# jw007123/hp-Adaptive-Signed-Distance-Field-Octree

Hardware: AMD Instinct MI355X
Metric: Query() Mpts/sec at targetError=1e-5 (union3 field, 10M SplitMix64 pts per GPU, HBM-resident); Create() ms reported as create_ms (higher is better)
Workload: dtype f64

## Files before the change

### hp-adaptive-signed-distance-field-octree_amd/csrc/fit.hip

```cpp
#include <hip/hip_runtime.h>

#include <algorithm>
#include <cstdint>
#include <cstdlib>

#include "device_types.hpp"
#include "fit_kernels.hpp"
#include "launch.hpp"
#include "leaf_eval.hpp"

namespace hpsdf {

__global__ __launch_bounds__(256) void pack_kernel(const PackItem* __restrict__ items, uint32_t nItems,
                                                   const double* __restrict__ arena, double* __restrict__ out) {
    const uint32_t wave = (blockIdx.x * blockDim.x + threadIdx.x) >> 6, lane = threadIdx.x & 63;
    if (wave >= nItems) return;
    const PackItem it = items[wave];
    for (uint32_t i = lane; i < it.count; i += 64) out[it.dst + i] = arena[it.src + i];
}

size_t fitLdsBytes(int degree, int nTasks, int planes) {
    const size_t nq = 4 * (size_t)degree + 1;
    return ((size_t)(degree + 1) * nq + 2 * nq + 8 * (size_t)nTasks + (size_t)nTasks * planes * nq * nq) * sizeof(double);
}
// ... 32 lines not shown
        sh.planes = std::max(sh.planes, std::min(nq, minPlanes));
        while (sh.cells > 1 && fitLdsBytes(degree, sh.cells, sh.planes) > kFitMaxLdsBytes) --sh.cells;
        sh.ldsBytes = fitLdsBytes(degree, sh.cells, sh.planes);
    }
    return sh;
}

#define HPSDF_DISPATCH_KIND(FN, field, ...)                          \
    switch ((field).kind) {                                          \
        case kFieldAnalytic: FN<kFieldAnalytic>(__VA_ARGS__); break; \
        case kFieldSamples: FN<kFieldSamples>(__VA_ARGS__); break;   \
        default: FN<kFieldMesh>(__VA_ARGS__); break;                 \
    }

hipError_t launchFitMulti(hipStream_t stream, const FitBlock* dBlocks, uint32_t maxBlocks, size_t ldsBytes, const FitTask* dTasks,
                          double* dArena, double* dErrs, const DeviceTables* dTables, const FieldDev& field, const RootMap& rm,
                          const uint32_t* dCount) {
    if (maxBlocks == 0) return hipSuccess;
    if (ldsBytes > kFitMaxLdsBytes) return hipErrorInvalidValue;
    HPSDF_DISPATCH_KIND(launchFitMultiKind, field, stream, dBlocks, maxBlocks, ldsBytes, dTasks, dArena, dErrs, dTables, field, rm, dCount);
    return hipGetLastError();
}

hipError_t launchFit(hipStream_t stream, int degree, int cellsPerThread, const FitBlock* dBlocks, uint32_t nBlocks,
                     size_t ldsBytes, const FitTask* dTasks, double* dArena, double* dErrs, double* dMirror,
                     const DeviceTables* dTables, const FieldDev& field, const RootMap& rm, const uint32_t* dRange) {
    if (nBlocks == 0) return hipSuccess;
    if (ldsBytes > kFitMaxLdsBytes) return hipErrorInvalidValue;
    HPSDF_DISPATCH_KIND(launchFitKind, field, stream, degree, cellsPerThread, dBlocks, nBlocks, ldsBytes, dTasks, dArena,
                        dErrs, dMirror, dTables, field, rm, dRange);
    return hipGetLastError();
}

hipError_t launchFieldEval(hipStream_t stream, const FieldDev& f, const DeviceTables* dTables, const double* dXyz,
                           size_t n, double* dOut) {
    if (n == 0) return hipSuccess;
    HPSDF_DISPATCH_KIND(launchFieldKind, f, stream, f, dTables, dXyz, n, dOut);
    return hipGetLastError();
}

hipError_t launchPack(hipStream_t stream, const PackItem* dItems, uint32_t nItems, const double* dArena, double* dOut) {
    if (nItems == 0) return hipSuccess;
    const unsigned blocks = (nItems + 3) / 4;
    hipLaunchKernelGGL(pack_kernel, dim3(blocks), dim3(256), 0, stream, dItems, nItems, dArena, dOut);
    return hipGetLastError();
}

}
```

### hp-adaptive-signed-distance-field-octree_amd/csrc/fit_analytic.hip

```cpp
#include "fit_kernels.hpp"

namespace hpsdf {

HPSDF_FIT_KIND_UNIT(, kFieldAnalytic)

}
```

### hp-adaptive-signed-distance-field-octree_amd/csrc/fit_kernels.hpp

```cpp
#pragma once
#include <hip/hip_runtime.h>

#include <cstdint>

#include "device_types.hpp"
#include "field_glue.hpp"
#include "launch.hpp"

namespace hpsdf {


constexpr int kFitPiece = 8;
#ifndef HPSDF_FIT_MIN_WAVES
#define HPSDF_FIT_MIN_WAVES 4
#endif

__device__ __forceinline__ double fitRowAny(double acc, double a1, const double* __restrict__ tk, double n2,
                                            const double* __restrict__ F, int nq) {
    int k = 0;
    for (; k + 4 <= nq; k += 4) {
        const double f0 = F[k], f1 = F[k + 1], f2 = F[k + 2], f3 = F[k + 3];
        const double t0 = tk[k], t1 = tk[k + 1], t2 = tk[k + 2], t3 = tk[k + 3];
        acc = acc + (a1 * t0 * n2) * f0;
        acc = acc + (a1 * t1 * n2) * f1;
        acc = acc + (a1 * t2 * n2) * f2;
        acc = acc + (a1 * t3 * n2) * f3;
    }
    for (; k < nq; ++k) acc = acc + (a1 * tk[k] * n2) * F[k];
    return acc;
}

template <int KIND, bool CSG, int DEG, int R, bool LEFT>
__device__ __forceinline__ void fitBlockBody(const FitBlock blk, const FitTask* __restrict__ tasks, double* __restrict__ arena,
                                             double* __restrict__ errs, double* __restrict__ mirror,
                                             const DeviceTables* __restrict__ T, const FieldDev& field, const RootMap& rm, double* lds) {
    static_assert(R == 1 || DEG > 0, "cell blocking needs a compile-time degree");
    __shared__ double sNl[13 * 11];
    __shared__ double sRec[26];
    __shared__ int32_t sMeshStack[kFitThreads / 64][kMeshStack];
    __shared__ unsigned char sPosI[KIND == kFieldMesh ? 64 : 4], sPosJK[KIND == kFieldMesh ? 64 : 4];
    const int tid = threadIdx.x;
    const int deg = DEG > 0 ? DEG : (int)blk.degree;
    const int nq = 4 * deg + 1, nq2 = nq * nq, G = blk.nTasks;
    const int rowStart = blk.rowStart, rowEnd = blk.rowEnd, nrows = rowEnd - rowStart;
    const int gl = nq * (nq - 1) / 2;
    const int planes = blk.planesPerChunk;
    const int depth = blk.depth;
    const bool split = blk.split != 0;

    double* sT = lds;
    double* sR = sT + (deg + 1) * nq;
    double* sW = sR + nq;
    double* sC = sW + nq;
    double* sF = sC + 8 * G;

    stageQueryTables(T, sNl, sRec);
    for (int q = tid; q < nq; q += kFitThreads) {
        const double x = T->roots[gl + q];
        sR[q] = x;
        sW[q] = T->weights[gl + q];
        double m2 = 0.0, m1 = 1.0;
        sT[q] = 1.0;
        for (int i = 1; i <= deg; ++i) {
            const double l = T->rec[i][0] * x * m1 - T->rec[i][1] * m2;
            m2 = m1, m1 = l;
// ... 189 lines not shown
    const int outBase = split ? 0 : stashBase;
    if (act0) {
#pragma unroll
        for (int r = 0; r < R; ++r)
            if (g2 + r < G) {
                const uint64_t at = tasks[blk.firstTask + g2 + r].outOff + (r0 - outBase);
                arena[at] = acc[r];
                if (mirror != nullptr) mirror[at] = acc[r];
                sF[(g2 + r) * stashStride + (r0 - stashBase)] = acc[r];
            }
    }
    if (act1) {
        arena[tasks[blk.firstTask].outOff + (r1 - outBase)] = acc1;
        sF[r1 - stashBase] = acc1;
    }
    if (weighted && rowStart > 0) {
        for (int s = tid; s < G * rowStart; s += kFitThreads) {
            const int g = s / rowStart, r = s - g * rowStart;
            const FitTask& tk = tasks[blk.firstTask + g];
            const double v = arena[tk.copyOff + r];
            arena[tk.outOff + r] = v;
            sF[g * stashStride + r] = v;
        }
    }
    __syncthreads();
    for (int g = tid; g < G; g += kFitThreads) {
        const int first = deg > 0 ? (int)T->count[deg - 1] : 0;
        double e = 0.0;
        for (int r = first > rowStart ? first : rowStart; r < rowEnd; ++r)
            if (T->bidx[r][3] == deg) {
                const double c = sF[g * stashStride + (r - stashBase)];
                e = e + c * c;
            }
        errs[tasks[blk.firstTask + g].errSlot] = e;
    }
}

template <int KIND, bool CSG, bool LEFT>
__global__ __launch_bounds__(kFitThreads, HPSDF_FIT_MIN_WAVES) void fit_multi_kernel(const FitBlock* __restrict__ blocks,
                                                                const FitTask* __restrict__ tasks, double* __restrict__ arena,
                                                                double* __restrict__ errs, const DeviceTables* __restrict__ T,
                                                                FieldDev field, RootMap rm, const uint32_t* __restrict__ count,
                                                                uint32_t countValue) {
    extern __shared__ double lds[];
    const uint32_t n = count ? *count : countValue;
    if (blockIdx.x >= n) return;
    const FitBlock blk = blocks[n - 1u - blockIdx.x];
    switch (blk.degree) {
        case 2: fitBlockBody<KIND, CSG, 2, 1, LEFT>(blk, tasks, arena, errs, nullptr, T, field, rm, lds); break;
        case 3: fitBlockBody<KIND, CSG, 3, 1, LEFT>(blk, tasks, arena, errs, nullptr, T, field, rm, lds); break;
        case 4: fitBlockBody<KIND, CSG, 4, 1, LEFT>(blk, tasks, arena, errs, nullptr, T, field, rm, lds); break;
        case 5: fitBlockBody<KIND, CSG, 5, 1, LEFT>(blk, tasks, arena, errs, nullptr, T, field, rm, lds); break;
        case 6: fitBlockBody<KIND, CSG, 6, 1, LEFT>(blk, tasks, arena, errs, nullptr, T, field, rm, lds); break;
        case 7: fitBlockBody<KIND, CSG, 7, 1, LEFT>(blk, tasks, arena, errs, nullptr, T, field, rm, lds); break;
        case 8: fitBlockBody<KIND, CSG, 8, 1, LEFT>(blk, tasks, arena, errs, nullptr, T, field, rm, lds); break;
        default: fitBlockBody<KIND, CSG, 0, 1, LEFT>(blk, tasks, arena, errs, nullptr, T, field, rm, lds); break;
    }
}

template <int KIND, bool CSG, int DEG, int R, bool LEFT>
__global__ __launch_bounds__(kFitThreads, HPSDF_FIT_MIN_WAVES) void fit_kernel(const FitBlock* __restrict__ blocks,
                                                          const FitTask* __restrict__ tasks, double* __restrict__ arena,
                                                          double* __restrict__ errs, double* __restrict__ mirror,
                                                          const DeviceTables* __restrict__ T, FieldDev field, RootMap rm,
                                                          const uint32_t* __restrict__ range) {
    extern __shared__ double lds[];
    uint32_t b = blockIdx.x;
    if (range != nullptr) {
// ... 22 lines not shown
                       const DeviceTables* dTables, const FieldDev& field, const RootMap& rm, const uint32_t* dRange) {
#define HPSDF_FIT_LAUNCH(D, RR)                                                                                       \
    hipLaunchKernelGGL((fit_kernel<KIND, CSG, D, RR, LEFT>), dim3(nBlocks), dim3(kFitThreads), ldsBytes, stream, dBlocks, \
                       dTasks, dArena, dErrs, dMeans, dTables, field, rm, dRange)
#define HPSDF_FIT_CASE(D)       \
    case D:                     \
        HPSDF_FIT_LAUNCH(D, 1); \
        break;
    if (cellsPerThread != 1 && cellsPerThread != 4) cellsPerThread = 1;
    switch (degree) {
        HPSDF_FIT_CASE(2)
        HPSDF_FIT_CASE(3)
        HPSDF_FIT_CASE(4)
        HPSDF_FIT_CASE(5)
        HPSDF_FIT_CASE(6)
        HPSDF_FIT_CASE(7)
        HPSDF_FIT_CASE(8)
        default:
            HPSDF_FIT_LAUNCH(0, 1);
    }
#undef HPSDF_FIT_CASE
#undef HPSDF_FIT_LAUNCH
}

template <int KIND, bool CSG, bool LEFT>
static void launchFitMultiT(hipStream_t stream, const FitBlock* dBlocks, uint32_t maxBlocks, size_t ldsBytes, const FitTask* dTasks,
                            double* dArena, double* dErrs, const DeviceTables* dTables, const FieldDev& field, const RootMap& rm,
                            const uint32_t* dCount) {
    hipLaunchKernelGGL((fit_multi_kernel<KIND, CSG, LEFT>), dim3(maxBlocks), dim3(kFitThreads), ldsBytes, stream, dBlocks, dTasks, dArena, dErrs,
                       dTables, field, rm, dCount, maxBlocks);
}

template <int KIND, bool CSG, bool LEFT>
static void launchFieldT(hipStream_t stream, const FieldDev& f, const DeviceTables* dTables, const double* dXyz,
                         size_t n, double* dOut) {
    hipLaunchKernelGGL((field_kernel<KIND, CSG, LEFT>), dim3(gridFor(n)), dim3(256), 0, stream, f, dTables, dXyz, n, dOut);
}

#define HPSDF_DISPATCH_FIELD_ORDER(FN, K, C, field, ...)  \
    do {                                                  \
        if ((field).leftAssoc) FN<K, C, true>(__VA_ARGS__); \
        else FN<K, C, false>(__VA_ARGS__);                \
    } while (0)
#define HPSDF_DISPATCH_FIELD(FN, K, field, ...)                                                  \
    do {                                                                                         \
        if ((field).csgOp >= 0) HPSDF_DISPATCH_FIELD_ORDER(FN, K, true, field, __VA_ARGS__);     \
        else HPSDF_DISPATCH_FIELD_ORDER(FN, K, false, field, __VA_ARGS__);                       \
    } while (0)

template <int KIND>
void launchFitKind(hipStream_t stream, int degree, int cellsPerThread, const FitBlock* dBlocks, uint32_t nBlocks, size_t ldsBytes,
                   const FitTask* dTasks, double* dArena, double* dErrs, double* dMirror, const DeviceTables* dTables,
                   const FieldDev& field, const RootMap& rm, const uint32_t* dRange) {
    HPSDF_DISPATCH_FIELD(launchFitT, KIND, field, stream, degree, cellsPerThread, dBlocks, nBlocks, ldsBytes, dTasks, dArena,
                         dErrs, dMirror, dTables, field, rm, dRange);
}
template <int KIND>
void launchFitMultiKind(hipStream_t stream, const FitBlock* dBlocks, uint32_t maxBlocks, size_t ldsBytes, const FitTask* dTasks,
                        double* dArena, double* dErrs, const DeviceTables* dTables, const FieldDev& field, const RootMap& rm,
                        const uint32_t* dCount) {
    HPSDF_DISPATCH_FIELD(launchFitMultiT, KIND, field, stream, dBlocks, maxBlocks, ldsBytes, dTasks, dArena, dErrs, dTables, field, rm, dCount);
}
template <int KIND>
void launchFieldKind(hipStream_t stream, const FieldDev& f, const DeviceTables* dTables, const double* dXyz, size_t n, double* dOut) {
    HPSDF_DISPATCH_FIELD(launchFieldT, KIND, f, stream, f, dTables, dXyz, n, dOut);
}
#undef HPSDF_DISPATCH_FIELD
#undef HPSDF_DISPATCH_FIELD_ORDER

#define HPSDF_FIT_KIND_UNIT(EXTERN, K)                                                                                                 \
    EXTERN template void launchFitKind<K>(hipStream_t, int, int, const FitBlock*, uint32_t, size_t, const FitTask*, double*, double*, \
                                          double*, const DeviceTables*, const FieldDev&, const RootMap&, const uint32_t*);            \
    EXTERN template void launchFitMultiKind<K>(hipStream_t, const FitBlock*, uint32_t, size_t, const FitTask*, double*, double*,      \
                                               const DeviceTables*, const FieldDev&, const RootMap&, const uint32_t*);                \
    EXTERN template void launchFieldKind<K>(hipStream_t, const FieldDev&, const DeviceTables*, const double*, size_t, double*);
HPSDF_FIT_KIND_UNIT(extern, kFieldAnalytic)
HPSDF_FIT_KIND_UNIT(extern, kFieldSamples)
HPSDF_FIT_KIND_UNIT(extern, kFieldMesh)

}
```

### hp-adaptive-signed-distance-field-octree_amd/csrc/fit_samples.hip

```cpp
#include "fit_kernels.hpp"

namespace hpsdf {

HPSDF_FIT_KIND_UNIT(, kFieldSamples)

}
```

### hp-adaptive-signed-distance-field-octree_amd/csrc/frontier.hip

```cpp
#include <hip/hip_runtime.h>

#include <algorithm>
#include <atomic>
#include <cfloat>
#include <cmath>
#include <cstddef>
#include <chrono>
#include <cstdio>
#include <cstdlib>
#include <cstring>
#include <memory>
#include <vector>

#include "builder.hpp"
#include "frontier.hpp"
#include "launch.hpp"
#include "runtime.hpp"

namespace hpsdf {

namespace {

constexpr uint32_t kFrJobs = 4096;
constexpr uint32_t kFrTasks = 9 * kFrJobs;
// ... 5 lines not shown
constexpr uint32_t kFrSort = 4096;
constexpr uint32_t kFrExact = 64;
constexpr uint32_t kFrStatusPad = 8;

struct FrHdr {
    uint32_t nNodes, nQueued, nJobs, done;
    uint32_t round, maxDegree, maxDepth, overflow;
    uint32_t nTasks, nBlocks, takenCount, candCount;
    uint32_t above;
    int32_t t1;
    uint32_t nLeaves, arrive;
    uint32_t degBlocks[13][2];
    uint32_t degTasks[13][2];
    uint32_t lowTasks[13][2];
    uint64_t arenaUsed, sampleUsed, nCoeffs, pad1;
    uint64_t jobs, pRefines, hRefines, dropped, fits, samples;
    uint64_t splitFits;
    uint32_t splitRound, padR;
    uint64_t roundBase, partStride;
    double total, target;
    uint32_t rP, rH, rD, rMaxDeg;
    uint32_t rOps, rPad;
    uint32_t sliceFirst[9];
    uint32_t padS;
    uint64_t packCount[8];
    uint64_t dbg[24];
    int64_t rCoeffDelta;
    double rTotal;
    uint32_t opsArrive, stuck;
    uint32_t chainStamp;
    uint32_t landed;
    uint32_t stored[2];
    uint32_t storeArrive[2];
    uint32_t hist1[2048];
    uint32_t hist2[2048];
    uint64_t agg[kFrJobs / 128];
};
constexpr size_t kFrHdrCopyBytes = offsetof(FrHdr, hist1);
static_assert(kFrHdrCopyBytes / 4 <= 1024, "frMirror copies the header with one thread a word");
static inline void frCpuRelax() {
#if defined(__x86_64__) || defined(__i386__)
    __builtin_ia32_pause();
#elif defined(__aarch64__)
    asm volatile("yield");
#endif
}

struct FrRound {
    uint32_t cCount[kFrClasses], cFirst[kFrClasses], cCursor[kFrClasses], cBlockFirst[kFrClasses], cBlocks[kFrClasses];
    uint64_t cArena[kFrClasses], cSample[kFrClasses];
    uint64_t cArenaO[8][kFrClasses];
    uint8_t cG[kFrClasses], cPlanes[kFrClasses];
    uint64_t arenaBase;
};

struct FrDev {
    FrHdr* hdr;
    FrHdr* hostHdr;
    FrRound* rnd;
    hpsdf_node* nodes;
    uint64_t* qErr;
    uint32_t* parent;
    uint64_t* segOff;
    uint8_t* segFirst;
    uint32_t* sub;
    uint32_t* taken;
// ... 1127 lines not shown
                        if (b + 2u < batches) {
                            FR_CHAIN_LOAD(ra, b + 2u)
                        }
                        __builtin_amdgcn_sched_barrier(0);
                        FR_CHAIN_ADD(rb)
                    }
                    if (b < batches) {
                        FR_CHAIN_ADD(ra)
                    }
#undef FR_CHAIN_LOAD
#undef FR_CHAIN_ADD
                    t = batches << 4;
                }
                for (; t < steps; ++t) total = __builtin_amdgcn_mfma_f64_4x4x4f64(mine[4u * t], 1.0, total, 0, 0, 0);
                q = steps << 2;
            }
            for (; q < n; ++q) total = total + src[q];
            if (d.stamps && tid == 0 && c0 == 0) d.hdr->dbg[16] = __builtin_readcyclecounter();
        }
        __syncthreads();
    }
    if (tid == 0) sOps[0] = total;
    __syncthreads();
    return sOps[0];
}

__device__ void frChainTotal(const FrDev& d, FrLds& L, bool chain0) {
    FrHdr* h = d.hdr;
    const uint32_t tid = threadIdx.x, wave = tid >> 6;
    if (wave != 0 && (wave & 3u) == 0) return;
    const uint32_t stamp = h->round + 1u;
    const bool round0 = stamp == 1u;
    double total = h->total;
    if (tid == 0) L.stuck = 0;
    __syncthreads();
    const uint32_t nJobs0 = h->nJobs;
    if (tid == 0) __hip_atomic_fetch_add(&h->arrive, 1u, __ATOMIC_RELAXED, __HIP_MEMORY_SCOPE_AGENT);
    if (round0 && !chain0) return;
    uint32_t nOps = nJobs0;
    if (!round0) {
        if (tid == 0 && !frWaitAtLeast(&h->opsArrive, gridDim.x - 2u)) L.stuck = 1;
        __syncthreads();
        nOps = frLoad(&h->rP) + 9u * frLoad(&h->rH);
        if (L.stuck) nOps = 0;
    }
    if (d.stamps && tid == 0) h->dbg[13] = __builtin_readcyclecounter();
    total = frRunChain(d, L, total, nOps, round0);
    if (tid == 0) {
        if (d.stamps) h->dbg[14] = __builtin_readcyclecounter();
        if (L.stuck) atomicExch(&h->stuck, 1u);
        h->rTotal = total;
        frRelease();
        __hip_atomic_store(&h->chainStamp, stamp, __ATOMIC_RELAXED, __HIP_MEMORY_SCOPE_AGENT);
    }
}

__device__ void frLeadRound(const FrDev& d, FrLds& L, int pre, bool chain0) {
    FrHdr* h = d.hdr;
    const uint32_t tid = threadIdx.x, nJobs = h->nJobs, round = h->round, stamp = round + 1u;
    const bool round0 = round == 0;
    const uint32_t nNodes0 = h->nNodes, nQ0 = h->nQueued;
    const uint64_t jobs0 = h->jobs, pRef0 = h->pRefines, hRef0 = h->hRefines, drop0 = h->dropped, nCoeffs0 = h->nCoeffs;
    const uint32_t nLeaves0 = h->nLeaves, maxDeg0 = h->maxDegree;
    const uint64_t fits0 = h->fits, samples0 = h->samples, arena0 = h->arenaUsed, split0 = h->splitFits;
    const double target = d.target;
    if (tid == 0) L.flag = 0, L.stuck = 0;
    if (tid == 0 && round0) {
        *(volatile uint32_t*)&d.hostHdr->landed = d.buildStamp;
        __threadfence_system();
    }
    __syncthreads();
    frPeerCheck(d, &L.flag);
    FR_STAMP(9);
    double total0 = 0.0;
    const bool ownChain = round0 && !chain0;
    if (ownChain) {
        if (d.stamps && tid == 0) h->dbg[13] = __builtin_readcyclecounter();
        total0 = frRunChain(d, L, h->total, nJobs, true);
        if (d.stamps && tid == 0) h->dbg[14] = __builtin_readcyclecounter();
    }
    if (tid == 0 && !frWaitAtLeast(&h->arrive, gridDim.x - 1u)) L.stuck = 1;
    __syncthreads();
    FR_STAMP(10);
    const uint32_t nP = frLoad(&h->rP), nH = frLoad(&h->rH), nD = frLoad(&h->rD), md = frLoad(&h->rMaxDeg);
    const long long cd = (long long)__hip_atomic_load(reinterpret_cast<unsigned long long*>(&h->rCoeffDelta), __ATOMIC_RELAXED, __HIP_MEMORY_SCOPE_AGENT);
    uint32_t overflow = frLoad(&h->overflow) | ((L.stuck || frLoad(&h->stuck)) ? 4u : 0u);
    const uint32_t nQ = nQ0 - (round0 ? 0u : nJobs) + nP + 8u * nH;
    const uint32_t nNodes = nNodes0 + 8u * nH;
    const bool stopsHere = ownChain && total0 < target;
    if (!stopsHere)
        for (uint32_t i = tid; i < 2048; i += 1024) L.hist[i] = frLoad(&h->hist1[i]);
    if (tid == 0) {
        const bool there = !ownChain && frLoad(&h->chainStamp) == stamp;
        if (there) frAcquire();
        L.c = (ownChain || there) ? 1u : 0u;
    }
    __syncthreads();
    bool haveTotal = L.c != 0;
    const bool canGoOn = nQ != 0 && overflow == 0;
    if (canGoOn && nQ > d.K && !stopsHere) {
        frThreshold(L.hist, d.K, L.tmp, &L.t, &L.above);
    } else {
        if (tid == 0) L.t = -1, L.above = nQ;
        __syncthreads();
    }
    const int T = L.t;
    const uint32_t above = L.above;
    auto awaitTotal = [&]() {
        if (tid == 0 && !frWaitAtLeast(&h->chainStamp, stamp)) L.stuck = 1;
        __syncthreads();
        if (L.stuck) overflow |= 4u;
    };
    const bool speculate = !haveTotal && pre && canGoOn;
    if (!haveTotal && !speculate) awaitTotal(), haveTotal = true;
    double total = 0.0;
    bool done = false;
    if (haveTotal) {
        if (ownChain) {
            total = total0;
        } else {
            total = *(volatile double*)&h->rTotal;
        }
        done = total < target || !canGoOn || overflow != 0;
    }
    if (tid == 0) {
        h->nQueued = nQ;
        h->nNodes = nNodes;
        h->jobs = jobs0 + nJobs, h->pRefines = pRef0 + nP, h->hRefines = hRef0 + nH, h->dropped = drop0 + nD;
        h->nLeaves = nLeaves0 + 7u * nH;
        h->nCoeffs = (uint64_t)((int64_t)nCoeffs0 + cd);
        if (md > maxDeg0) h->maxDegree = md;
        h->round = stamp;
        h->takenCount = 0, h->candCount = 0;
        h->rPad = L.flag;
        h->t1 = T, h->above = above;
    }
    FR_STAMP(11);
    __syncthreads();
    if (pre && !done) {
        for (uint32_t i = tid; i < 2048; i += 1024) L.hist[i] = 0;
        if (tid == 0) L.c = 0, L.next = 0;
        __syncthreads();
        {
            const int lane = (int)(tid & 63);
            for (uint32_t base = 0; base < nNodes; base += 1024u) {
                const uint32_t i = base + tid;
                const uint64_t bits = i < nNodes ? d.qErr[i] : kNotQueued;
                const bool queued = bits != kNotQueued;
                const int d0 = (int)frDigit(0, bits, i);
                const bool take = queued && d0 > T, cand = queued && d0 == T;
                const unsigned long long mt = __ballot(take), mc = __ballot(cand);
// ... 258 lines not shown
    if (threadIdx.x != 0 || blockIdx.x != 0) return;
    volatile uint32_t* f = d.hostFlag;
    f[0] = d.hdr->nJobs;
    __threadfence_system();
    f[1] = stamp;
    __threadfence_system();
}
__global__ __launch_bounds__(256) void fr_weigh_kernel(FrDev d, uint32_t stride, uint32_t base, uint32_t count) {
    const FrHdr* h = d.hdr;
    if (h->done) return;
    const uint32_t i = blockIdx.x * 256u + threadIdx.x;
    if (i >= count) return;
    if (stride == 1u && i % 9u != 0u) return;
    d.errs[base + i] = d.errs[base + i] * d.weights[base + i];
}

struct FrTemplate {
    const hpsdf_node* nodes;
    const uint32_t* parent;
    const uint32_t* sub;
    uint32_t nNodes, nLeaves, nTasks, nBlocks;
    uint64_t arenaRows, samples;
    uint32_t sliceFirst[9];
};
__global__ __launch_bounds__(256) void fr_init_kernel(FrDev d, FrTemplate t) {
    const uint32_t i = blockIdx.x * 256u + threadIdx.x;
    if (i < t.nNodes) {
        d.nodes[i] = t.nodes[i];
        d.parent[i] = t.parent[i];
        d.sub[i] = 0;
        d.qErr[i] = kNotQueued;
        d.segFirst[i] = 2;
    }
    if (blockIdx.x != 0) return;
    if (threadIdx.x == 0 && d.world > 1) *frStatusSlot(d, d.rank) = 0.0;
    uint32_t* hw = reinterpret_cast<uint32_t*>(d.hdr);
    for (uint32_t w = threadIdx.x; w < sizeof(FrHdr) / 4; w += 256u) hw[w] = 0;
    __syncthreads();
    if (threadIdx.x == 0) {
        FrHdr* h = d.hdr;
        h->nNodes = t.nNodes;
        h->nJobs = t.nLeaves;
        h->nLeaves = t.nLeaves;
        h->t1 = -1;
        h->total = 4096.0 * HPSDF_INITIAL_NODE_ERR;
        h->maxDegree = 2;
        h->nTasks = t.nTasks, h->nBlocks = t.nBlocks;
        h->degTasks[2][0] = 0, h->degTasks[2][1] = t.nTasks;
        h->degBlocks[2][0] = 0, h->degBlocks[2][1] = t.nBlocks;
        h->arenaUsed = t.arenaRows;
        h->sampleUsed = t.samples;
        h->fits = t.nTasks, h->samples = t.samples;
        h->nCoeffs = (uint64_t)t.nLeaves * frCoef(2);
        for (int r = 0; r < 9; ++r) h->sliceFirst[r] = t.sliceFirst[r];
    }
    if (d.world > 1)
        for (uint32_t j = threadIdx.x; j < t.nLeaves; j += 256u) {
            uint32_t o = 0;
            for (int r = 1; r < d.world; ++r) o += t.sliceFirst[r] <= j ? 1u : 0u;
            d.jobOwner[j] = (uint8_t)o;
        }
}

}

struct FrontierWorkspace {
// ... 642 lines not shown
            if (*roundWord != want) {
                HPSDF_HIP(hipMemcpy(ws->hostHdr, d.hdr, kFrHdrCopyBytes, hipMemcpyDeviceToHost));
                if (hh->round != want) return fail(HPSDF_ERR_STATE, "frontier: a round ended without advancing");
            }
        }
        std::atomic_thread_fence(std::memory_order_acquire);
        tSync += now() - ts;
        return HPSDF_OK;
    };

    d.errStride = stride0, d.errStrideNext = strideK;
    d.buildStamp = ++ws->buildStamp ? ws->buildStamp : ++ws->buildStamp;
    d.stamps = trace ? 1u : 0u;
    ws->hostHdr->round = 0, ws->hostHdr->done = 0;
    auto initDev = [&] {
        FrDev di = d;
        di.errStride = stride0;
        return di;
    };
    {
        hipError_t e = ws->ensureArena(std::max<uint64_t>(1, T0.arenaRows), 0, s);
        if (e == hipSuccess && mesh) e = ws->ensureSamples(std::max<uint64_t>(1, T0.samples), s);
        if (e != hipSuccess) return hipFail(e, "frontier buffers");
        if ((rc = prepareNext(T.nNodes, T0.arenaRows, 2u, 0))) return rc;
        d.target = cfg.target_error_threshold;
        if (!ws->clean || ws->cleanRank != rank || ws->cleanWorld != world) FR_LAUNCH(fr_init_kernel, dim3((T.nNodes + 255) / 256), dim3(256), s, initDev(), T0);
        ws->clean = false;
        FieldDev fdr = fd;
        if (mesh) {
            HPSDF_HIP(launchMeshSample(s, r0Tasks, T0.nTasks, 2, ctx->dTables, fd, rm, ws->samples));
            fdr.kind = kFieldSamples;
            fdr.samples = ws->samples;
        }
        HPSDF_HIP(launchFit(s, 2, 1, r0Blocks, T0.nBlocks, r0Lds, r0Tasks, ws->arena, d.errs, world == 1 ? ws->pinnedDev : nullptr, ctx->dTables, fdr, rm));
        if (weighted && (rc = applyWeights(r0Blocks, T0.nBlocks, r0Lds, r0Tasks, nullptr, true, world == 1 ? 0u : (uint32_t)rank * stride0,
                                           T0.sliceFirst[rank + 1] - T0.sliceFirst[rank])))
            return rc;
        if (replica) {
            if (arenaPartBytes != (size_t)part0 * sizeof(double)) return fail(HPSDF_ERR_STATE, "frontier: round 0's part of the arena");
            partPending = false;
            if ((rc = exchange(ws->arena, arenaPartBytes, "round 0's rows"))) return rc;
        }
        if ((rc = exchange(d.errs, (size_t)stride0 * sizeof(double), "round 0"))) return rc;
        phase = 0;
        d.errStride = strideK;
    }
    int rounds = 0;
    uint32_t knownNodes = T.nNodes, knownMaxDeg = 2;
    uint64_t knownArena = T0.arenaRows;
    for (;;) {
        const bool pre = (uint64_t)knownNodes + 8ull * Kj <= inlineNodes;
        const bool splitCur = splitOpen, tooLargeCur = samplesTooLarge;
        FrDev dk = d;
        dk.splitFit = splitCur ? std::max(2, ctx->splitMinDegree) : 0;
        if (rounds == 0) {
            dk.batchIdx = ws->tmplLeaves, dk.batchErr = ws->tmplErr, dk.jobP = r0JobP, dk.jobH = r0JobP;
            dk.errStride = stride0;
        }
        FR_LAUNCH(fr_round_kernel, dim3(2 + ((rounds == 0 ? T.nLeaves : Kj) + 127u) / 128u), dim3(1024), s, dk, (pre ? 1 : 0) | (ws->lastWentOn && pre ? 2 : 0));
        const bool noBlind = std::getenv("HPSDF_FRONTIER_NO_BLIND") != nullptr;
        const bool blind = (rounds >= 1 || ws->lastWentOn) && pre && world == 1 && !weighted && !frSyncEveryLaunch() && !noBlind;
        if (blind) {
            if (mesh && tooLargeCur) return fail(HPSDF_ERR_UNSUPPORTED, "round too large for the sampled mesh path");
            d.splitFit = dk.splitFit;
            FrDev de = d;
            FR_LAUNCH(fr_emit_kernel, dim3((Kj + 127u) / 128u), dim3(1024), s, de);
// ... 6 lines not shown
                std::memcpy(early, &nc0, 8);
                std::memcpy(early + 8 + 8 * (size_t)nc0, &nn0, 8);
                std::memcpy(early + 16 + 8 * (size_t)nc0, ws->hostNodesAfterRound0.data(), sizeof(hpsdf_node) * (size_t)nn0);
                std::memcpy(early + 16 + 8 * (size_t)nc0 + sizeof(hpsdf_node) * (size_t)nn0, &cfg, sizeof cfg);
                const volatile uint32_t* landed = &hh->landed;
                const volatile uint32_t* roundWord = &hh->round;
                const double limit = now() + 2.0e3;
                while (*landed != d.buildStamp && *roundWord == 0 && now() < limit) frCpuRelax();
                if (*landed == d.buildStamp) {
                    std::atomic_thread_fence(std::memory_order_acquire);
                    const size_t total = 8 * (size_t)nc0, piece = 32768;
                    size_t at = 0;
                    for (; at < total && (*roundWord == 0 || *(const volatile uint32_t*)&hh->done); at += piece) std::memcpy(early + 8 + at, ws->pinned + at, std::min(piece, total - at));
                    earlyCopied = at >= total;
                }
            }
        }
        if ((rc = waitForRound((uint32_t)rounds + 1u))) return rc;
        ++rounds;
        if (world > 1 && hh->rPad)
            return fail(HPSDF_ERR_STATE, "rank " + std::to_string(hh->rPad - 1) + " failed in round " + std::to_string(rounds - 1) + ": its own error was returned there");
        if (hh->overflow & 1u) return fail(HPSDF_ERR_STATE, "frontier: node capacity exceeded");
        if (hh->overflow & 4u) return fail(HPSDF_ERR_STATE, "frontier: a workgroup of the round's kernel did not arrive");
        if (trace) {
            std::fprintf(stderr, "[frontier round %d] lead (cycles): wait-all %lld close %lld", rounds - 1, (long long)(hh->dbg[10] - hh->dbg[9]),
                         (long long)(hh->dbg[11] - hh->dbg[10]));
            if (!hh->done && pre) {
                std::fprintf(stderr, " | select %lld batch", (long long)(hh->dbg[0] - hh->dbg[11]));
                for (int k = 1; k <= 8; ++k) std::fprintf(stderr, " %lld", (long long)(hh->dbg[k] - hh->dbg[k - 1]));
                std::fprintf(stderr, " | total+commit %lld", (long long)(hh->dbg[12] - hh->dbg[8]));
            }
            std::fprintf(stderr, " | chain %lld (first operands %lld, first 2048 additions %lld)", (long long)(hh->dbg[14] - hh->dbg[13]), (long long)(hh->dbg[15] - hh->dbg[13]),
                         (long long)(hh->dbg[16] - hh->dbg[15]));
            std::fprintf(stderr, "\n");
        }
        if (rounds == 1 && world == 1 && hh->done && early && hh->nCoeffs == T.arenaRows && hh->nNodes == T.nNodes) {
            if (!earlyCopied) std::memcpy(early + 8, ws->pinned, 8 * (size_t)T.arenaRows);
            hipLaunchKernelGGL(fr_init_kernel, dim3((T.nNodes + 255) / 256), dim3(256), 0, s, initDev(), T0);
            ws->clean = hipGetLastError() == hipSuccess, ws->cleanRank = rank, ws->cleanWorld = world;
            ws->lastWentOn = false;
            *block = early;
            *size = 8 + 8 * (size_t)T.arenaRows + 8 + sizeof(hpsdf_node) * (size_t)T.nNodes + sizeof(hpsdf_config);
            early = nullptr;
            if (stats) {
                std::memset(stats, 0, sizeof *stats);
                stats->rounds = hh->round, stats->jobs = hh->jobs, stats->p_refines = hh->pRefines, stats->h_refines = hh->hRefines;
                stats->dropped = hh->dropped, stats->fits = hh->fits, stats->samples = hh->samples;
                stats->n_nodes = hh->nNodes, stats->n_leaves = hh->nLeaves, stats->n_coeffs = hh->nCoeffs, stats->total_error = hh->total;
                stats->fit_mode = (uint64_t)ctx->fitMode, stats->split_fits = hh->splitFits, stats->device_frontier = 1;
            }
            if (trace) std::fprintf(stderr, "[frontierCreate] us: total %.0f (waiting for the device %.0f, stopped after round 0)\n", now() - t0, tSync);
            return HPSDF_OK;
        }
        ctx->freeBlock(early);
        early = nullptr;
        if (hh->done) break;
        if (!(std::fabs(hh->total) <= DBL_MAX))
            return fail(HPSDF_ERR_INVALID_ARGUMENT, "the field is not a finite number at some sample point (the build's total error is NaN or infinite)");
        knownNodes = hh->nNodes, knownMaxDeg = hh->maxDegree, knownArena = hh->arenaUsed;
        if (world > 1) phase = 2;
        if (replica && pre) partPending = true, partOff = hh->roundBase, arenaPartBytes = (size_t)hh->partStride * sizeof(double);
        if (!pre) {
            FrDev dl = d;
            dl.splitFit = dk.splitFit;
            FR_LAUNCH(fr_select_kernel, dim3(std::min<uint32_t>(512u, (knownNodes + 255u) / 256u)), dim3(256), s, dl);
            FR_LAUNCH(fr_batch_kernel, dim3(1), dim3(1024), s, dl);
// ... 113 lines not shown
```

### hp-adaptive-signed-distance-field-octree_amd/csrc/launch.hpp

```cpp
#pragma once
#include <algorithm>
#include <vector>
#include <hip/hip_runtime_api.h>

#include <cstddef>
#include <cstdint>
#include <cstdlib>

#include "device_types.hpp"

namespace hpsdf {

constexpr unsigned kQueryMaxGrid = 256 * 8 * 4;
constexpr size_t kQueryFewPoints = 256;
inline unsigned gridFor(size_t n) {
    size_t blocks = (n + 255) / 256;
    static const size_t capEnv = [] { const char* e = std::getenv("HPSDF_QUERY_GRID"); return e ? (size_t)std::max(1, std::atoi(e)) : (size_t)0; }();
    const size_t cap = capEnv ? capEnv : kQueryMaxGrid;
    return (unsigned)(blocks < 1 ? 1 : (blocks > cap ? cap : blocks));
}
hipError_t launchQuery(hipStream_t stream, const TreeDev& t, const DeviceTables* dTables, const double* dXyz, size_t n,
                       double* dOut, double* dGrad, bool allInline, uint32_t* dDeferCount, uint32_t* dDeferIdx);
hipError_t launchQueryRay(hipStream_t stream, const TreeDev& t, const DeviceTables* dTables, const double* dOrigins,
                          const double* dDirs, const double* dTMax, size_t n, uint8_t* dHit, double* dT);
hipError_t launchQueryLattice(hipStream_t stream, const TreeDev& t, const DeviceTables* dTables, const SurfaceLattice& g, double* dOut);
hipError_t launchSlicePoints(hipStream_t stream, double c, float minX, float minY, float step, uint32_t nSamples,
                             double* dXyz);
hipError_t launchFitWeight(hipStream_t stream, const FitBlock* dBlocks, uint32_t nBlocks, size_t ldsBytes, const FitTask* dTasks,
                           const double* dArena, double* dMeans, const DeviceTables* dTables, const uint32_t* dCount = nullptr);
hipError_t launchQueryTrueGradient(hipStream_t stream, const TreeDev& t, const DeviceTables* dTables, const double* dXyz, size_t n,
                                   uint32_t flags, double* dOut, double* dGrad, bool allInline);
constexpr size_t kFitMaxLdsBytes = 60 * 1024;
constexpr int kFitBlockThreads = 256;
constexpr int kFitThreads = 256;
constexpr size_t kFitChunkLdsBytes = 40 * 1024;
size_t fitLdsBytes(int degree, int nTasks, int planes);
struct FitShape {
    int cells;
    int cellsPerThread;
    int planes;
    size_t ldsBytes;
};
FitShape fitShape(int degree, int nrows, uint32_t count, bool weighted, bool latencyBound = false);
hipError_t launchFit(hipStream_t stream, int degree, int cellsPerThread, const FitBlock* dBlocks, uint32_t nBlocks, size_t ldsBytes,
                     const FitTask* dTasks, double* dArena, double* dErrs, double* dMirror,
                     const DeviceTables* dTables, const FieldDev& field, const RootMap& rm, const uint32_t* dRange = nullptr);
hipError_t launchFitMulti(hipStream_t stream, const FitBlock* dBlocks, uint32_t maxBlocks, size_t ldsBytes, const FitTask* dTasks,
                          double* dArena, double* dErrs, const DeviceTables* dTables, const FieldDev& field, const RootMap& rm,
                          const uint32_t* dCount);
hipError_t launchFieldEval(hipStream_t stream, const FieldDev& f, const DeviceTables* dTables, const double* dXyz,
                           size_t n, double* dOut);
hipError_t launchPack(hipStream_t stream, const PackItem* dItems, uint32_t nItems, const double* dArena, double* dOut);
hipError_t launchMeshSample(hipStream_t stream, const FitTask* dTasks, uint32_t nTasks, int degree, const DeviceTables* dTables,
                            const FieldDev& field, const RootMap& rm, double* dSamples);
hipError_t launchMeshSampleRange(hipStream_t stream, const FitTask* dTasks, const uint32_t* dRange, uint32_t maxTasks, int degree,
                                 const DeviceTables* dTables, const FieldDev& field, const RootMap& rm, double* dSamples);
constexpr int kMfmaCells = 16;
bool fitMfmaSupports(int degree, const FieldDev& field);
hipError_t launchFitMfma(hipStream_t stream, int degree, const FitBlock* dBlocks, uint32_t nBlocks, const FitTask* dTasks, double* dArena,
                         double* dErrs, const DeviceTables* dTables, const FieldDev& field, const RootMap& rm, const uint32_t* dRange = nullptr);
int fitSplitDefaultMinDegree();
bool fitSplitSupports(int degree, int minDegree);
hipError_t launchFitLow(hipStream_t stream, int degree, const FitTask* dTasks, const uint32_t* dRange, uint32_t first, uint32_t count,
                        uint32_t maxTasks, double* dArena, const DeviceTables* dTables, const double* dSamples);
hipError_t launchFitMfmaLow(hipStream_t stream, int degree, const FitTask* dTasks, const uint32_t* dRange, uint32_t first, uint32_t count,
                            uint32_t maxTasks, double* dArena, const DeviceTables* dTables, const double* dSamples, const RootMap& rm, int leftAssoc);
hipError_t launchMeshEvalWave(hipStream_t stream, const FieldDev& f, const double* dXyz, size_t n, double* dOut);
void meshEvalHostPoints(const MeshDev& hm, const double* xyz, size_t n, double* out);
hipError_t launchMeshNaive(hipStream_t stream, const FieldDev& f, const double* dXyz, size_t n, double* dOut, unsigned long long* dKeys = nullptr);
hipError_t launchAcosfSelftest(hipStream_t stream, uint32_t first, uint32_t stride, size_t n, float* dOut);
constexpr int kTriRecordFloats = 12;
constexpr int kTriPreFloats = 12;
hipError_t launchMeshTriPos(hipStream_t stream, const float* dVerts, const uint32_t* dTris, uint64_t nTris, float* dTriPos,
                            const uint32_t* dSlotTri, float* dTriPre);
hipError_t sortPairsU32(hipStream_t stream, void* tmp, size_t& tmpBytes, const uint32_t* keys, uint32_t* keysOut, const uint32_t* vals, uint32_t* valsOut,
                        size_t n, unsigned bits);
hipMemPool_t meshPool(int dev);
void meshPoolTrim(int dev);
constexpr uint64_t kCgChunk = 256;
// ... 48 lines not shown
```

Before: 94170.

## Fold round-0 error total into the fit launch via an extra consumer block

Adds a round-0 fit kernel with one extra block that spin-waits on per-leaf error slots, published with atomic stores and pre-seeded with a sentinel. As the other blocks finish, it accumulates the total with f64 MFMA adds, double-buffered through LDS, and publishes it with a stamp. The frontier kernel then reuses this total and skips its own serial chain of additions for round 0. This targets Create() latency only, at the cost of a block that busy-waits on others and depends on forward progress. The Query throughput metric should be unaffected.

New measurement: 93960 (median of 2 runs). No clear change (-0.2%).

```diff
diff --git a/hp-adaptive-signed-distance-field-octree_amd/csrc/fit.hip b/hp-adaptive-signed-distance-field-octree_amd/csrc/fit.hip
--- a/hp-adaptive-signed-distance-field-octree_amd/csrc/fit.hip
+++ b/hp-adaptive-signed-distance-field-octree_amd/csrc/fit.hip
@@ -88,6 +88,22 @@
     return hipGetLastError();
 }
 
+hipError_t launchFitRound0(hipStream_t stream, const FitBlock* dBlocks, uint32_t nBlocks, size_t ldsBytes, const FitTask* dTasks, double* dArena,
+                           double* dErrs, double* dMirror, const DeviceTables* dTables, const FieldDev& field, const RootMap& rm,
+                           const Round0Total& rt) {
+    if (nBlocks == 0 || ldsBytes > kFitMaxLdsBytes || ldsBytes < kRound0TotalLdsBytes) return hipErrorInvalidValue;
+    switch (field.kind) {
+        case kFieldAnalytic:
+            launchFitRound0Kind<kFieldAnalytic>(stream, dBlocks, nBlocks, ldsBytes, dTasks, dArena, dErrs, dMirror, dTables, field, rm, rt);
+            break;
+        case kFieldSamples:
+            launchFitRound0Kind<kFieldSamples>(stream, dBlocks, nBlocks, ldsBytes, dTasks, dArena, dErrs, dMirror, dTables, field, rm, rt);
+            break;
+        default: return hipErrorInvalidValue;
+    }
+    return hipGetLastError();
+}
+
 hipError_t launchFieldEval(hipStream_t stream, const FieldDev& f, const DeviceTables* dTables, const double* dXyz,
                            size_t n, double* dOut) {
     if (n == 0) return hipSuccess;
diff --git a/hp-adaptive-signed-distance-field-octree_amd/csrc/fit_analytic.hip b/hp-adaptive-signed-distance-field-octree_amd/csrc/fit_analytic.hip
--- a/hp-adaptive-signed-distance-field-octree_amd/csrc/fit_analytic.hip
+++ b/hp-adaptive-signed-distance-field-octree_amd/csrc/fit_analytic.hip
@@ -3,5 +3,6 @@
 namespace hpsdf {
 
 HPSDF_FIT_KIND_UNIT(, kFieldAnalytic)
+HPSDF_FIT_ROUND0_UNIT(, kFieldAnalytic)
 
 }
diff --git a/hp-adaptive-signed-distance-field-octree_amd/csrc/fit_kernels.hpp b/hp-adaptive-signed-distance-field-octree_amd/csrc/fit_kernels.hpp
--- a/hp-adaptive-signed-distance-field-octree_amd/csrc/fit_kernels.hpp
+++ b/hp-adaptive-signed-distance-field-octree_amd/csrc/fit_kernels.hpp
@@ -30,7 +30,7 @@
     return acc;
 }
 
-template <int KIND, bool CSG, int DEG, int R, bool LEFT>
+template <int KIND, bool CSG, int DEG, int R, bool LEFT, bool PUBLISH = false>
 __device__ __forceinline__ void fitBlockBody(const FitBlock blk, const FitTask* __restrict__ tasks, double* __restrict__ arena,
                                              double* __restrict__ errs, double* __restrict__ mirror,
                                              const DeviceTables* __restrict__ T, const FieldDev& field, const RootMap& rm, double* lds) {
@@ -286,8 +286,121 @@
                 const double c = sF[g * stashStride + (r - stashBase)];
                 e = e + c * c;
             }
-        errs[tasks[blk.firstTask + g].errSlot] = e;
-    }
+        if constexpr (PUBLISH)
+            __hip_atomic_store(&errs[tasks[blk.firstTask + g].errSlot], e, __ATOMIC_RELAXED, __HIP_MEMORY_SCOPE_AGENT);
+        else
+            errs[tasks[blk.firstTask + g].errSlot] = e;
+    }
+}
+
+constexpr uint32_t kRound0Chunk = 512;
+static_assert(kRound0Chunk <= 3u * (kFitThreads - 64) && kRound0Chunk % 64u == 0 && 2 * kRound0Chunk * sizeof(double) == kRound0TotalLdsBytes,
+              "three waves of loaders, whole batches of sixteen MFMA steps, the launcher's LDS check");
+__device__ __forceinline__ void fitRound0Total(const Round0Total& rt, double* lds) {
+    __shared__ uint32_t sGaveUp;
+    const uint32_t tid = threadIdx.x, wave = tid >> 6, lane = tid & 63u;
+    const bool adder = wave == 0;
+    const uint32_t ltid = tid - 64u;
+    if (tid == 0) sGaveUp = 0;
+    const unsigned long long t0 = wall_clock64();
+    if (rt.dbg && tid == 0) rt.dbg[0] = __builtin_readcyclecounter();
+    auto loadChunk = [&](uint32_t first, double* dst) {
+        uint32_t pending = 0;
+#pragma unroll
+        for (int u = 0; u < 3; ++u) {
+            const uint32_t k = ltid + (uint32_t)u * 192u;
+            if (k < kRound0Chunk && first + k < rt.nOps) pending |= 1u << u;
+        }
+        while (pending) {
+            double v[3];
+#pragma unroll
+            for (int u = 0; u < 3; ++u) {
+                const uint32_t k = first + ltid + (uint32_t)u * 192u;
+                v[u] = (pending >> u) & 1u ? __hip_atomic_load(&rt.errs[(size_t)k * rt.errStride], __ATOMIC_RELAXED, __HIP_MEMORY_SCOPE_AGENT) : 0.0;
+            }
+#pragma unroll
+            for (int u = 0; u < 3; ++u) {
+                const uint32_t k = ltid + (uint32_t)u * 192u;
+                if (((pending >> u) & 1u) && (unsigned long long)__double_as_longlong(v[u]) != kRound0NotYet) {
+                    dst[k] = v[u] - rt.batchErr[first + k];
+                    pending &= ~(1u << u);
+                }
+            }
+            if (pending) {
+                __builtin_amdgcn_s_sleep(8);
+                if (wall_clock64() - t0 > rt.waitTicks) {
+                    atomicExch(&sGaveUp, 1u);
+                    break;
+                }
+            }
+        }
+    };
+    double total = *rt.total0;
+    __syncthreads();
+    if (!adder) loadChunk(0, lds);
+    __syncthreads();
+    bool gaveUp = sGaveUp != 0;
+    for (uint32_t c0 = 0, half = 0; c0 < rt.nOps && !gaveUp; c0 += kRound0Chunk, half ^= 1u) {
+        __syncthreads();
+        const uint32_t n = rt.nOps - c0 < kRound0Chunk ? rt.nOps - c0 : kRound0Chunk;
+        if (!adder) {
+            if (c0 + kRound0Chunk < rt.nOps) loadChunk(c0 + kRound0Chunk, lds + (half ^ 1u) * kRound0Chunk);
+        } else {
+            const double* src = lds + half * kRound0Chunk;
+            const double* mine = src + (lane >> 4);
+            const uint32_t steps = n >> 2, batches = steps >> 4;
+            uint32_t t = 0;
+            if (batches) {
+                double ra[16], rb[16];
+#define HPSDF_R0_LOAD(r, batch) \
+    _Pragma("unroll") for (int u = 0; u < 16; ++u) r[u] = mine[4u * (16u * (batch) + (uint32_t)u)];
+#define HPSDF_R0_ADD(r) \
+    _Pragma("unroll") for (int u = 0; u < 16; ++u) total = __builtin_amdgcn_mfma_f64_4x4x4f64(r[u], 1.0, total, 0, 0, 0);
+                HPSDF_R0_LOAD(ra, 0u)
+                uint32_t b = 0;
+                for (; b + 2u <= batches; b += 2u) {
+                    HPSDF_R0_LOAD(rb, b + 1u)
+                    __builtin_amdgcn_sched_barrier(0);
+                    HPSDF_R0_ADD(ra)
+                    if (b + 2u < batches) {
+                        HPSDF_R0_LOAD(ra, b + 2u)
+                    }
+                    __builtin_amdgcn_sched_barrier(0);
+                    HPSDF_R0_ADD(rb)
+                }
+                if (b < batches) {
+                    HPSDF_R0_ADD(ra)
+                }
+#undef HPSDF_R0_LOAD
+#undef HPSDF_R0_ADD
+                t = batches << 4;
+            }
+            for (; t < steps; ++t) total = __builtin_amdgcn_mfma_f64_4x4x4f64(mine[4u * t], 1.0, total, 0, 0, 0);
+            for (uint32_t q = steps << 2; q < n; ++q) total = total + src[q];
+        }
+        __syncthreads();
+        gaveUp = sGaveUp != 0;
+    }
+    if (tid == 0 && !gaveUp) {
+        *rt.outTotal = total;
+        __builtin_amdgcn_fence(__ATOMIC_RELEASE, "agent");
+        asm volatile("s_waitcnt vmcnt(0)" ::: "memory");
+        __hip_atomic_store(rt.outStamp, rt.stamp, __ATOMIC_RELAXED, __HIP_MEMORY_SCOPE_AGENT);
+        if (rt.dbg) rt.dbg[1] = __builtin_readcyclecounter();
+    }
+}
+
+template <int KIND, bool CSG, bool LEFT>
+__global__ __launch_bounds__(kFitThreads, HPSDF_FIT_MIN_WAVES) void fit_round0_kernel(const FitBlock* __restrict__ blocks,
+                                                                 const FitTask* __restrict__ tasks, double* __restrict__ arena,
+                                                                 double* errs, double* __restrict__ mirror,
+                                                                 const DeviceTables* __restrict__ T, FieldDev field, RootMap rm, Round0Total rt) {
+    extern __shared__ double lds[];
+    if (blockIdx.x + 1u == gridDim.x) {
+        fitRound0Total(rt, lds);
+        return;
+    }
+    fitBlockBody<KIND, CSG, 2, 1, LEFT, true>(blocks[blockIdx.x], tasks, arena, errs, mirror, T, field, rm, lds);
 }
 
 template <int KIND, bool CSG, bool LEFT>
@@ -376,6 +489,14 @@
 }
 
 template <int KIND, bool CSG, bool LEFT>
+static void launchFitRound0T(hipStream_t stream, const FitBlock* dBlocks, uint32_t nBlocks, size_t ldsBytes, const FitTask* dTasks, double* dArena,
+                             double* dErrs, double* dMirror, const DeviceTables* dTables, const FieldDev& field, const RootMap& rm,
+                             const Round0Total& rt) {
+    hipLaunchKernelGGL((fit_round0_kernel<KIND, CSG, LEFT>), dim3(nBlocks + 1u), dim3(kFitThreads), ldsBytes, stream, dBlocks, dTasks, dArena, dErrs,
+                       dMirror, dTables, field, rm, rt);
+}
+
+template <int KIND, bool CSG, bool LEFT>
 static void launchFieldT(hipStream_t stream, const FieldDev& f, const DeviceTables* dTables, const double* dXyz,
                          size_t n, double* dOut) {
     hipLaunchKernelGGL((field_kernel<KIND, CSG, LEFT>), dim3(gridFor(n)), dim3(256), 0, stream, f, dTables, dXyz, n, dOut);
@@ -406,6 +527,12 @@
     HPSDF_DISPATCH_FIELD(launchFitMultiT, KIND, field, stream, dBlocks, maxBlocks, ldsBytes, dTasks, dArena, dErrs, dTables, field, rm, dCount);
 }
 template <int KIND>
+void launchFitRound0Kind(hipStream_t stream, const FitBlock* dBlocks, uint32_t nBlocks, size_t ldsBytes, const FitTask* dTasks, double* dArena,
+                         double* dErrs, double* dMirror, const DeviceTables* dTables, const FieldDev& field, const RootMap& rm,
+                         const Round0Total& rt) {
+    HPSDF_DISPATCH_FIELD(launchFitRound0T, KIND, field, stream, dBlocks, nBlocks, ldsBytes, dTasks, dArena, dErrs, dMirror, dTables, field, rm, rt);
+}
+template <int KIND>
 void launchFieldKind(hipStream_t stream, const FieldDev& f, const DeviceTables* dTables, const double* dXyz, size_t n, double* dOut) {
     HPSDF_DISPATCH_FIELD(launchFieldT, KIND, f, stream, f, dTables, dXyz, n, dOut);
 }
@@ -421,5 +548,10 @@
 HPSDF_FIT_KIND_UNIT(extern, kFieldAnalytic)
 HPSDF_FIT_KIND_UNIT(extern, kFieldSamples)
 HPSDF_FIT_KIND_UNIT(extern, kFieldMesh)
-
-}
+#define HPSDF_FIT_ROUND0_UNIT(EXTERN, K)                                                                                                    \
+    EXTERN template void launchFitRound0Kind<K>(hipStream_t, const FitBlock*, uint32_t, size_t, const FitTask*, double*, double*, double*, \
+                                                const DeviceTables*, const FieldDev&, const RootMap&, const Round0Total&);
+HPSDF_FIT_ROUND0_UNIT(extern, kFieldAnalytic)
+HPSDF_FIT_ROUND0_UNIT(extern, kFieldSamples)
+
+}
diff --git a/hp-adaptive-signed-distance-field-octree_amd/csrc/fit_samples.hip b/hp-adaptive-signed-distance-field-octree_amd/csrc/fit_samples.hip
--- a/hp-adaptive-signed-distance-field-octree_amd/csrc/fit_samples.hip
+++ b/hp-adaptive-signed-distance-field-octree_amd/csrc/fit_samples.hip
@@ -3,5 +3,6 @@
 namespace hpsdf {
 
 HPSDF_FIT_KIND_UNIT(, kFieldSamples)
+HPSDF_FIT_ROUND0_UNIT(, kFieldSamples)
 
 }
diff --git a/hp-adaptive-signed-distance-field-octree_amd/csrc/frontier.hip b/hp-adaptive-signed-distance-field-octree_amd/csrc/frontier.hip
--- a/hp-adaptive-signed-distance-field-octree_amd/csrc/frontier.hip
+++ b/hp-adaptive-signed-distance-field-octree_amd/csrc/frontier.hip
@@ -61,6 +61,8 @@
     uint32_t landed;
     uint32_t stored[2];
     uint32_t storeArrive[2];
+    double r0Total;
+    uint32_t r0Stamp, padT;
     uint32_t hist1[2048];
     uint32_t hist2[2048];
     uint64_t agg[kFrJobs / 128];
@@ -1254,11 +1256,12 @@
     const uint32_t stamp = h->round + 1u;
     const bool round0 = stamp == 1u;
     double total = h->total;
+    const bool have0 = round0 && frLoad(&h->r0Stamp) == d.buildStamp;
     if (tid == 0) L.stuck = 0;
     __syncthreads();
     const uint32_t nJobs0 = h->nJobs;
     if (tid == 0) __hip_atomic_fetch_add(&h->arrive, 1u, __ATOMIC_RELAXED, __HIP_MEMORY_SCOPE_AGENT);
-    if (round0 && !chain0) return;
+    if (round0 && (!chain0 || have0)) return;
     uint32_t nOps = nJobs0;
     if (!round0) {
         if (tid == 0 && !frWaitAtLeast(&h->opsArrive, gridDim.x - 2u)) L.stuck = 1;
@@ -1295,7 +1298,11 @@
     frPeerCheck(d, &L.flag);
     FR_STAMP(9);
     double total0 = 0.0;
-    const bool ownChain = round0 && !chain0;
+    const bool have0 = round0 && frLoad(&h->r0Stamp) == d.buildStamp;
+    const bool ownChain = round0 && !chain0 && !have0;
+    if (have0)
+        total0 = __longlong_as_double((long long)__hip_atomic_load(reinterpret_cast<const unsigned long long*>(&h->r0Total), __ATOMIC_RELAXED, __HIP_MEMORY_SCOPE_AGENT));
+    const bool known0 = ownChain || have0;
     if (ownChain) {
         if (d.stamps && tid == 0) h->dbg[13] = __builtin_readcyclecounter();
         total0 = frRunChain(d, L, h->total, nJobs, true);
@@ -1309,13 +1316,13 @@
     uint32_t overflow = frLoad(&h->overflow) | ((L.stuck || frLoad(&h->stuck)) ? 4u : 0u);
     const uint32_t nQ = nQ0 - (round0 ? 0u : nJobs) + nP + 8u * nH;
     const uint32_t nNodes = nNodes0 + 8u * nH;
-    const bool stopsHere = ownChain && total0 < target;
+    const bool stopsHere = known0 && total0 < target;
     if (!stopsHere)
         for (uint32_t i = tid; i < 2048; i += 1024) L.hist[i] = frLoad(&h->hist1[i]);
     if (tid == 0) {
-        const bool there = !ownChain && frLoad(&h->chainStamp) == stamp;
+        const bool there = !known0 && frLoad(&h->chainStamp) == stamp;
         if (there) frAcquire();
-        L.c = (ownChain || there) ? 1u : 0u;
+        L.c = (known0 || there) ? 1u : 0u;
     }
     __syncthreads();
     bool haveTotal = L.c != 0;
@@ -1338,7 +1345,7 @@
     double total = 0.0;
     bool done = false;
     if (haveTotal) {
-        if (ownChain) {
+        if (known0) {
             total = total0;
         } else {
             total = *(volatile double*)&h->rTotal;
@@ -1663,6 +1670,7 @@
         d.qErr[i] = kNotQueued;
         d.segFirst[i] = 2;
     }
+    if (d.world == 1 && i < t.nLeaves) reinterpret_cast<unsigned long long*>(d.errs)[(size_t)i * HPSDF_JOB_HEADER_DOUBLES] = kRound0NotYet;
     if (blockIdx.x != 0) return;
     if (threadIdx.x == 0 && d.world > 1) *frStatusSlot(d, d.rank) = 0.0;
     uint32_t* hw = reinterpret_cast<uint32_t*>(d.hdr);
@@ -2371,6 +2379,16 @@
             fdr.kind = kFieldSamples;
             fdr.samples = ws->samples;
         }
+        const bool total0InLaunch = world == 1 && !weighted && r0Lds >= kRound0TotalLdsBytes && std::getenv("HPSDF_FRONTIER_NO_ROUND0_TOTAL") == nullptr;
+        if (total0InLaunch) {
+            Round0Total rt{};
+            rt.errs = d.errs, rt.batchErr = ws->tmplErr, rt.total0 = &d.hdr->total;
+            rt.outTotal = &d.hdr->r0Total, rt.outStamp = &d.hdr->r0Stamp;
+            rt.dbg = trace ? reinterpret_cast<unsigned long long*>(&d.hdr->dbg[17]) : nullptr;
+            rt.waitTicks = kFrWaitTicks;
+            rt.nOps = T.nLeaves, rt.errStride = HPSDF_JOB_HEADER_DOUBLES, rt.stamp = d.buildStamp;
+            HPSDF_HIP(launchFitRound0(s, r0Blocks, T0.nBlocks, r0Lds, r0Tasks, ws->arena, d.errs, ws->pinnedDev, ctx->dTables, fdr, rm, rt));
+        } else
         HPSDF_HIP(launchFit(s, 2, 1, r0Blocks, T0.nBlocks, r0Lds, r0Tasks, ws->arena, d.errs, world == 1 ? ws->pinnedDev : nullptr, ctx->dTables, fdr, rm));
         if (weighted && (rc = applyWeights(r0Blocks, T0.nBlocks, r0Lds, r0Tasks, nullptr, true, world == 1 ? 0u : (uint32_t)rank * stride0,
                                            T0.sliceFirst[rank + 1] - T0.sliceFirst[rank])))
@@ -2443,6 +2461,7 @@
             }
             std::fprintf(stderr, " | chain %lld (first operands %lld, first 2048 additions %lld)", (long long)(hh->dbg[14] - hh->dbg[13]), (long long)(hh->dbg[15] - hh->dbg[13]),
                          (long long)(hh->dbg[16] - hh->dbg[15]));
+            if (rounds == 1 && hh->r0Stamp == d.buildStamp) std::fprintf(stderr, " | total in the fit launch %lld", (long long)(hh->dbg[18] - hh->dbg[17]));
             std::fprintf(stderr, "\n");
         }
         if (rounds == 1 && world == 1 && hh->done && early && hh->nCoeffs == T.arenaRows && hh->nNodes == T.nNodes) {
diff --git a/hp-adaptive-signed-distance-field-octree_amd/csrc/launch.hpp b/hp-adaptive-signed-distance-field-octree_amd/csrc/launch.hpp
--- a/hp-adaptive-signed-distance-field-octree_amd/csrc/launch.hpp
+++ b/hp-adaptive-signed-distance-field-octree_amd/csrc/launch.hpp
@@ -45,6 +45,21 @@
 hipError_t launchFit(hipStream_t stream, int degree, int cellsPerThread, const FitBlock* dBlocks, uint32_t nBlocks, size_t ldsBytes,
                      const FitTask* dTasks, double* dArena, double* dErrs, double* dMirror,
                      const DeviceTables* dTables, const FieldDev& field, const RootMap& rm, const uint32_t* dRange = nullptr);
+constexpr unsigned long long kRound0NotYet = 0xBFF0000000000000ull;
+constexpr size_t kRound0TotalLdsBytes = 2 * 512 * sizeof(double);
+struct Round0Total {
+    const double* errs;
+    const double* batchErr;
+    const double* total0;
+    double* outTotal;
+    uint32_t* outStamp;
+    unsigned long long* dbg;
+    unsigned long long waitTicks;
+    uint32_t nOps, errStride, stamp, pad;
+};
+hipError_t launchFitRound0(hipStream_t stream, const FitBlock* dBlocks, uint32_t nBlocks, size_t ldsBytes, const FitTask* dTasks, double* dArena,
+                           double* dErrs, double* dMirror, const DeviceTables* dTables, const FieldDev& field, const RootMap& rm,
+                           const Round0Total& rt);
 hipError_t launchFitMulti(hipStream_t stream, const FitBlock* dBlocks, uint32_t maxBlocks, size_t ldsBytes, const FitTask* dTasks,
                           double* dArena, double* dErrs, const DeviceTables* dTables, const FieldDev& field, const RootMap& rm,
                           const uint32_t* dCount);
```
